# suyashk12/hipgp

Measured on NVIDIA B200. Metric: toeplitz_matvec_GBps_in_pcg_1e6grid, higher is better.
Workload: dtype f32

## Files before the change

hipgp_b200/csrc/conv_kernels.cuh:

```cuda
#pragma once
#include "fft_engine.cuh"

namespace hipgp {

enum RowsFwdMode { RF_PLAIN = 0, RF_PUPDATE = 1, RF_XRUPDATE = 2, RF_SELFDOT = 3 };
enum RowsInvMode { RI_PLAIN = 0, RI_DOT = 1 };
enum DotKind { DOT_PAP = 0, DOT_ZR = 1, DOT_RR = 2 };
enum ColsMode { CM_FWD = 0, CM_INV = 1, CM_FUSED = 2 };
enum SpecKind { SPEC_NONE = 0, SPEC_REAL = 1, SPEC_CPLX = 2, SPEC_CPLX_CONJ = 3 };

struct PcgDev {
    double* zr;
    double* zr_prev;
    double* pAp;
    double* rr;
    const double* rr_all;
    double* partial;
    unsigned* row_cnt;
    unsigned* rhs_cnt;
    int* flags;
    double tol;
    int B;
    int cg_mode;
};
// ... 33 lines not shown
                st.row_cnt[b] = 0;
                if (kind == DOT_PAP) st.pAp[b] = v;
                else if (kind == DOT_ZR) { st.zr_prev[b] = st.zr[b]; st.zr[b] = v; }
                else {
                    st.rr[b] = v;
                    if (st.cg_mode) { st.zr_prev[b] = st.zr[b]; st.zr[b] = v; }
                }
                __threadfence();
                if (kind == DOT_RR) {
                    const unsigned nb = atomicAdd(st.rhs_cnt, 1u) + 1u;
                    if (nb == (unsigned)st.B) {
                        __threadfence();
                        bool all = true;
                        const volatile double* rr = st.rr_all ? st.rr_all : st.rr;
                        for (int i = 0; i < st.B; ++i) all = all && (sqrt(rr[i]) < st.tol);
                        st.rhs_cnt[0] = 0;
                        st.flags[1] += 1;
                        st.flags[2] = 0;
                        if (all) st.flags[0] = 1;
                    }
                }
            }
        }
    }
}

template <class T>
struct RowsParams {
    const T* in;
    T* out;
    T* v0;
    T* v1;
    const T* v2;
    cplx<T>* W;
    long total_rows;
    int nrows;
    int n_real;
    int L, H;
    long W_pitch;
    int W_rows;
    LineFft<T> f;
    const cplx<T>* twL;
    const cplx<T>* twLp;
    const int* part;
    const int* pairq;
    const int* pairs; const cplx<T>* pairw; int npair0;
    const int* quadq; const cplx<T>* quadw; int nquad;
    int RB, RBP;
    int mode, dot_kind, do_fft;
    int vec_ok;
    int vec16_ok;
    int tma_ok;
    int tma_op;
    const void* spec; int spec_kind;
    PcgDev st;
};

template <class T>
__global__ void __launch_bounds__(256) rows_fwd_kernel(RowsParams<T> P) {
    HIPGP_DYN_SMEM(smem_raw);
    cplx<T>* s = reinterpret_cast<cplx<T>*>(smem_raw);
    const int tid = threadIdx.x, nthreads = blockDim.x;
    const int warp = tid >> 5, lane = tid & 31, nwarps = nthreads >> 5;
    if (P.mode != RF_PLAIN && P.st.flags[0]) return;
    const long g0 = (long)blockIdx.x * P.RB;
    const long g1 = g0 + P.RB < P.total_rows ? g0 + P.RB : P.total_rows;
    const int nl = (int)(g1 - g0);
    const int H = P.H, RBP = P.RBP, n = P.n_real;

    for (int line = warp; line < P.RB; line += nwarps) {
        if (line >= nl) {
            if (P.do_fft) for (int k = lane; k < H; k += 32) s[(size_t)k * RBP + line] = mk<T>(0, 0);
            continue;
        }
        const long g = g0 + line;
        const int b = (int)(g / P.nrows);
        const size_t off = (size_t)g * n;
        T acc = 0;
        T coef = 0;
        bool first = false;
        if (P.mode == RF_PUPDATE) {
            first = P.st.flags[2] != 0;
            coef = first ? (T)0 : (T)(P.st.zr[b] / P.st.zr_prev[b]);
        } else if (P.mode == RF_XRUPDATE) {
            coef = (T)(P.st.zr[b] / P.st.pAp[b]);
        }
        for (int k = lane; k < H; k += 32) {
            T e[2];
#pragma unroll
            for (int h = 0; h < 2; ++h) {
                const int i = 2 * k + h;
                T val = 0;
                if (i < n) {
                    if (P.mode == RF_PLAIN) {
                        val = P.in[off + i];
                    } else if (P.mode == RF_PUPDATE) {
                        const T z = P.in[off + i];
                        val = first ? z : z + coef * P.v0[off + i];
                        P.v0[off + i] = val;
                    } else if (P.mode == RF_SELFDOT) {
                        val = P.in[off + i];
                        acc += val * val;
                    } else {
                        const T pv = P.v2[off + i];
                        P.v1[off + i] = P.v1[off + i] + coef * pv;
                        val = P.v0[off + i] - coef * P.in[off + i];
// ... 193 lines not shown
```

hipgp_b200/csrc/fast_kernels.cuh:

```cuda
#pragma once
#include "lane_fft.cuh"

namespace hipgp {

template <class T> __device__ __forceinline__ void ld2(const T* p, bool vec, T& a, T& b, bool ok0, bool ok1) {
    if (vec && ok1) { const cplx<T> t = ld_stream(reinterpret_cast<const cplx<T>*>(p)); a = t.x; b = t.y; }
    else { a = ok0 ? ld_stream(p) : (T)0; b = ok1 ? ld_stream(p + 1) : (T)0; }
}
template <class T> __device__ __forceinline__ void st2(T* p, bool vec, T a, T b, bool ok0, bool ok1) {
    if (vec && ok1) { st_stream(reinterpret_cast<cplx<T>*>(p), mk<T>(a, b)); }
    else { if (ok0) st_stream(p, a); if (ok1) st_stream(p + 1, b); }
}

__device__ __forceinline__ double team_sum(double v, int tw) {
    for (int o = tw >> 1; o > 0; o >>= 1) v += __shfl_xor_sync(0xffffffffu, v, o);
    return v;
}

__device__ __forceinline__ Lane<float> lane_spec(Lane<float> v, const void* spec, int kind, size_t idx) {
    if (kind == SPEC_REAL) {
        const cplx<float> sv = ld_stream(reinterpret_cast<const cplx<float>*>(reinterpret_cast<const float*>(spec) + idx));
        return lmul_real2(v, sv.x, sv.y);
    }
    const cplx<float>* sp = reinterpret_cast<const cplx<float>*>(spec) + idx;
    const cplx<float> w0 = ld_stream(sp), w1 = ld_stream(sp + 1);
    return kind == SPEC_CPLX ? lmul_cplx2<false>(v, w0, w1) : lmul_cplx2<true>(v, w0, w1);
}
__device__ __forceinline__ Lane<double> lane_spec(Lane<double> v, const void* spec, int kind, size_t idx) {
    if (kind == SPEC_REAL) return lscale(v, ld_stream(reinterpret_cast<const double*>(spec) + idx));
    const cplx<double> w = ld_stream(reinterpret_cast<const cplx<double>*>(spec) + idx);
    return kind == SPEC_CPLX ? lmul(v, w) : lmulc(v, w);
}
__device__ __forceinline__ Lane<float> lane_spec_smem(Lane<float> v, const void* p) {
    const float2 s2 = *reinterpret_cast<const float2*>(p);
    Lane<float> r; r.re = __fmul2_rn(v.re, s2); r.im = __fmul2_rn(v.im, s2); return r;
}
__device__ __forceinline__ Lane<double> lane_spec_smem(Lane<double> v, const void* p) { return lscale(v, *reinterpret_cast<const double*>(p)); }

template <class T, int NL, int NT, int MINB, int R0, int... Rs>
__global__ void __launch_bounds__(NT, MINB) cols_fast_kernel(ColsParams<T> P) {
    using G = TileGeo<T, NL, R0, Rs...>;
    constexpr int Ln = G::Ln, NST = G::NST, RLAST = G::RLAST, LPT = LaneInfo<T>::LPT, TBL = NL * LPT, S0 = Ln / R0;
    HIPGP_DYN_SMEM(smem_raw);
    Lane<T>* s = reinterpret_cast<Lane<T>*>(smem_raw);
    const int tid = threadIdx.x;
    if (P.done_flag && *P.done_flag) return;
    const int mode = P.mode;
    const size_t pitch = (size_t)P.pitch;
    const size_t spitch = P.spec_pitch ? (size_t)P.spec_pitch : (size_t)P.pitch;
    const long ntiles = (long)P.nx * P.ny * P.nz;
    auto tile_origin = [&](long t, long& c0, size_t& ioff, size_t& ooff) {
        long bx, by, bz;
        if (P.batch_fastest) { bz = t % P.nz; const long r = t / P.nz; bx = r % P.nx; by = r / P.nx; }
        else { bx = t % P.nx; const long r = t / P.nx; by = r % P.ny; bz = r / P.ny; }
// ... 464 lines not shown
            if (tid < nl) { double a = 0.0; for (int k = 0; k < WPR; ++k) a += s_part[tid * WPR + k]; P.st.partial[g0 + tid] = a; }
        }
    }
    __syncthreads();
    if (want_dot) pcg_finalize(P.st, mode == RF_XRUPDATE ? DOT_RR : DOT_ZR, g0, g1, P.nrows, tid, NT);

    {
        const bool zero_hi = is_pow2(R0) && R0 > 1 && (n + 1) / 2 <= H / 2;
        const cplx<T>* tw0 = P.f.twst + P.f.twoff[0];
#pragma unroll 1
        for (int it = tid; it < S0 * NL; it += NT) {
            const int lane = it % NL, j = it / NL;
            cplx<T> w[R0];
            if (NST > 1) lane_twiddles<R0, S0>(w, tw0, j);
            const T* srow0 = side + (size_t)(lane * LPT) * SROW;
            const T* srow1 = side + (size_t)(lane * LPT + LPT - 1) * SROW;
            const bool ok0 = lane * LPT < nl, ok1 = lane * LPT + LPT - 1 < nl;
            auto elem = [&](int r) -> Lane<T> {
                const int i = 2 * (j + r * S0);
                const bool in_row = i < SROW;
                const cplx<T> e0 = (ok0 && in_row) ? *reinterpret_cast<const cplx<T>*>(srow0 + i) : mk<T>(0, 0);
                const cplx<T> e1 = (LPT == 2 && ok1 && in_row) ? *reinterpret_cast<const cplx<T>*>(srow1 + i) : mk<T>(0, 0);
                return lane_make(e0, e1);
            };
            Lane<T> v[R0];
            if (zero_hi) {
#pragma unroll
                for (int r = 0; r < R0 / 2; ++r) v[r] = elem(r);
                lbfly_zero_hi<R0, T>(v);
            } else {
#pragma unroll
                for (int r = 0; r < R0; ++r) v[r] = elem(r);
                lbfly<R0, false, T>(v);
            }
            if (NST > 1) {
#pragma unroll
                for (int r = 1; r < R0; ++r) v[r] = lmul(v[r], w[r]);
            }
            Lane<T>* base = s + (G::slot(j) * NL + lane);
#pragma unroll
            for (int r = 0; r < R0; ++r) base[r * LEG0] = v[r];
        }
    }
    __syncthreads();

    if constexpr (NST > 1) {
        LaneMidFwd<G, T, NL, NT, H / R0, 1, Rs...>::run(s, P.f, tid);
        lane_stage<G, T, NL, NT, RLAST, RLAST, false>(s, P.f.twst, tid);
        __syncthreads();
    }

    constexpr int NPAIR0 = NST > 1 ? RLAST / 2 + 1 : H / 2 + 1;
    constexpr int NQUAD = NST > 1 ? (H - RLAST) / 4 : 0;
#pragma unroll 1
    for (int it = tid; it < NPAIR0 * NL; it += NT) {
        const int lane = it % NL, pi = it / NL;
        const QuadIdx pq = reinterpret_cast<const QuadIdx*>(P.pairs)[pi];
        const int q = pq.a, q2 = pq.b;
        Lane<T> Xa, Xb;
        bool two;
        if (q == 0) {
            const Lane<T> z = s[lane];
            Lane<T> zs; zs.re = z.im; zs.im = z.re;
            Xa = lscale(z + zs, (T)2); Xb = lscale(z - zs, (T)2);
            Xa.im = lzero<T>().im; Xb.im = lzero<T>().im;
            two = true;
        } else {
            const cplx<T> wq = ldg_c(P.pairw + pi);
            const Lane<T> a = s[G::slot(q) * NL + lane], c = lconj(s[G::slot(q2) * NL + lane]);
            const Lane<T> E = a + c;
            const Lane<T> t = lmul(lmi<false>(a - c), wq);
            Xa = E + t; Xb = lconj(E - t);
            two = q2 != q;
        }
#pragma unroll
        for (int l = 0; l < LPT; ++l) {
            const int row = lane * LPT + l;
            if (row < nl) {
                cplx<T>* dst = P.W + s_wbase[row];
                WRow<T>::store1(dst, q, lane_get(Xa, l));
                if (two) WRow<T>::store1(dst, q2, lane_get(Xb, l));
            }
        }
    }
    if constexpr (NQUAD > 0) {
        constexpr int QIT = (NQUAD * NL + NT - 1) / NT;
        QuadIdx qq[QIT]; cplx<T> wa[QIT], wa1[QIT];
#pragma unroll
        for (int k = 0; k < QIT; ++k) {
            const int it = tid + k * NT, qi = it / NL;
            if (it < NQUAD * NL) { qq[k] = reinterpret_cast<const QuadIdx*>(P.quadq)[qi]; wa[k] = ldg_c(P.quadw + 2 * qi); wa1[k] = ldg_c(P.quadw + 2 * qi + 1); }
        }
#pragma unroll
        for (int k = 0; k < QIT; ++k) {
            const int it = tid + k * NT, lane = it % NL;
            if (it < NQUAD * NL) {
                const Lane<T>* pa = s + (G::slot(qq[k].a) * NL + lane);
                const Lane<T>* pb = s + (G::slot(qq[k].b) * NL + lane);
                const Lane<T> za = pa[0], za1 = pa[NL], zb = pb[0], zb1 = pb[NL];
                Lane<T> c = lconj(zb1);
                Lane<T> E = za + c;
                Lane<T> t = lmul(lmi<false>(za - c), wa[k]);
                const Lane<T> Xa = E + t, Xb1 = lconj(E - t);
                c = lconj(zb);
                E = za1 + c;
                t = lmul(lmi<false>(za1 - c), wa1[k]);
                const Lane<T> Xa1 = E + t, Xb = lconj(E - t);
                const bool self = qq[k].a == qq[k].b;
#pragma unroll
                for (int l = 0; l < LPT; ++l) {
                    const int row = lane * LPT + l;
                    if (row < nl) {
                        cplx<T>* dst = P.W + s_wbase[row];
                        if (self) WRow<T>::store2(dst, qq[k].a, lane_get(Xa, l), lane_get(Xb1, l));
                        else { WRow<T>::store2(dst, qq[k].a, lane_get(Xa, l), lane_get(Xa1, l)); WRow<T>::store2(dst, qq[k].b, lane_get(Xb, l), lane_get(Xb1, l)); }
                    }
                }
            }
        }
    }
#ifndef HIPGP_EMU
    if (bulk_store_pending && tid == 0) asm volatile("cp.async.bulk.wait_group.read 0;" ::: "memory");
#endif
}

template <class T, int NL, int NT, int MINB, int R0, int... Rs>
__global__ void __launch_bounds__(NT, MINB) rows_inv_fast_kernel(RowsParams<T> P) {
    using G = TileGeo<T, NL, R0, Rs...>;
    constexpr int H = G::Ln, NST = G::NST, RLAST = G::RLAST, LPT = LaneInfo<T>::LPT, NROW = NL * LPT, S0 = H / R0;
    constexpr int LEG0 = G::leg(NST > 1 ? S0 : 1);
    HIPGP_DYN_SMEM(smem_raw);
    Lane<T>* s = reinterpret_cast<Lane<T>*>(smem_raw);
    const int tid = threadIdx.x;
    if (P.mode != RI_PLAIN && P.st.flags[0]) return;
    const long g0 = (long)blockIdx.x * NROW;
    const long g1 = g0 + NROW < P.total_rows ? g0 + NROW : P.total_rows;
    const int nl = (int)(g1 - g0);
    const int n = P.n_real;

    __shared__ long s_wbase[32];
    __shared__ double s_part[32];
    if (tid < NROW && tid < nl) {
        const long gr = g0 + tid;
        const long b = gr / P.nrows;
        s_wbase[tid] = (b * P.W_rows + (gr - b * P.nrows)) * P.W_pitch;
    }
    __syncthreads();

    const int spec_kind = P.spec_kind;
    constexpr int NPAIR0 = NST > 1 ? RLAST / 2 + 1 : H / 2 + 1;
    constexpr int NQUAD = NST > 1 ? (H - RLAST) / 4 : 0;
#pragma unroll 1
    for (int it = tid; it < NPAIR0 * NL; it += NT) {
        const int lane = it % NL, pi = it / NL;
        const QuadIdx pq = reinterpret_cast<const QuadIdx*>(P.pairs)[pi];
        const int q = pq.a, q2 = pq.b;
        const cplx<T> wq = ldg_c(P.pairw + pi);
        cplx<T> ya[LPT], yc[LPT];
#pragma unroll
        for (int l = 0; l < LPT; ++l) {
            const int row = lane * LPT + l;
            ya[l] = mk<T>(0, 0); yc[l] = mk<T>(0, 0);
            if (row < nl) {
                const cplx<T>* src = P.W + s_wbase[row];
                ya[l] = WRow<T>::load1(src, q); yc[l] = WRow<T>::load1(src, q2);
                if (spec_kind != SPEC_NONE) { ya[l] = apply_spec(ya[l], P.spec, spec_kind, (size_t)q); yc[l] = apply_spec(yc[l], P.spec, spec_kind, (size_t)q2); }
            }
        }
        const Lane<T> a = lane_make(ya[0], ya[LPT - 1]);
        Lane<T> c = lane_make(yc[0], yc[LPT - 1]);
        if (q == 0) {
            Lane<T> z; z.re = (a + c).re; z.im = (a - c).re;
            s[lane] = z;
        } else {
            c = lconj(c);
            const Lane<T> E = a + c;
            const Lane<T> iO = lmi<true>(lmulc(a - c, wq));
            s[G::slot(q) * NL + lane] = E + iO;
            if (q2 != q) s[G::slot(q2) * NL + lane] = lconj(E - iO);
        }
    }
    if constexpr (NQUAD > 0) {
        constexpr int QIT = (NQUAD * NL + NT - 1) / NT;
        QuadIdx qq[QIT]; cplx<T> wa[QIT], wa1[QIT];
        cplx<T> ya[QIT][LPT], ya1[QIT][LPT], yb[QIT][LPT], yb1[QIT][LPT];
#pragma unroll
        for (int k = 0; k < QIT; ++k) {
            int it = tid + k * NT;
            it = it < NQUAD * NL ? it : NQUAD * NL - 1;
            const int qi = it / NL;
            qq[k] = reinterpret_cast<const QuadIdx*>(P.quadq)[qi]; wa[k] = ldg_c(P.quadw + 2 * qi); wa1[k] = ldg_c(P.quadw + 2 * qi + 1);
        }
#pragma unroll
        for (int k = 0; k < QIT; ++k) {
            int it = tid + k * NT;
            it = it < NQUAD * NL ? it : NQUAD * NL - 1;
            const int lane = it % NL;
#pragma unroll
            for (int l = 0; l < LPT; ++l) {
                const int row = lane * LPT + l;
                const cplx<T>* src = P.W + s_wbase[row < nl ? row : nl - 1];
                WRow<T>::load2(src, qq[k].a, ya[k][l], ya1[k][l]);
                WRow<T>::load2(src, qq[k].b, yb[k][l], yb1[k][l]);
            }
        }
#pragma unroll
        for (int k = 0; k < QIT; ++k) {
            const int it = tid + k * NT, lane = it % NL;
            if (it < NQUAD * NL) {
                const bool self = qq[k].a == qq[k].b;
                if (spec_kind != SPEC_NONE) {
#pragma unroll
                    for (int l = 0; l < LPT; ++l) {
                        ya[k][l] = apply_spec(ya[k][l], P.spec, spec_kind, (size_t)qq[k].a); ya1[k][l] = apply_spec(ya1[k][l], P.spec, spec_kind, (size_t)qq[k].a + 1);
                        yb[k][l] = apply_spec(yb[k][l], P.spec, spec_kind, (size_t)qq[k].b); yb1[k][l] = apply_spec(yb1[k][l], P.spec, spec_kind, (size_t)qq[k].b + 1);
                    }
                }
                const Lane<T> A = lane_make(ya[k][0], ya[k][LPT - 1]), A1 = lane_make(ya1[k][0], ya1[k][LPT - 1]);
                const Lane<T> Bn = lane_make(yb[k][0], yb[k][LPT - 1]), B1 = lane_make(yb1[k][0], yb1[k][LPT - 1]);
                Lane<T>* pa = s + (G::slot(qq[k].a) * NL + lane);
                Lane<T>* pb = s + (G::slot(qq[k].b) * NL + lane);
                Lane<T> c = lconj(B1);
                Lane<T> E = A + c;
                Lane<T> iO = lmi<true>(lmulc(A - c, wa[k]));
                pa[0] = E + iO;
                pb[NL] = lconj(E - iO);
                if (!self) {
                    c = lconj(Bn);
                    E = A1 + c;
                    iO = lmi<true>(lmulc(A1 - c, wa1[k]));
                    pa[NL] = E + iO;
                    pb[0] = lconj(E - iO);
                }
            }
        }
    }
    __syncthreads();

    if constexpr (NST > 1) {
        lane_stage<G, T, NL, NT, RLAST, RLAST, true>(s, P.f.twst, tid);
        __syncthreads();
        LaneMidInv<G, T, NL, NT, H / R0, 1, Rs...>::run(s, P.f, tid);
    }

    const int SROW = (n + 3) & ~3;
    T* side = reinterpret_cast<T*>(smem_raw + G::smem_bytes());
    const bool want_dot = P.mode == RI_DOT;
    {
        const bool out_lo = is_pow2(R0) && R0 > 1 && (n + 1) / 2 <= H / 2;
        const cplx<T>* tw0 = P.f.twst + P.f.twoff[0];
#pragma unroll 1
        for (int it = tid; it < S0 * NL; it += NT) {
            const int lane = it % NL, j = it / NL;
            cplx<T> w[R0];
            if (NST > 1) lane_twiddles<R0, S0>(w, tw0, j);
            const Lane<T>* base = s + (G::slot(j) * NL + lane);
            Lane<T> v[R0];
#pragma unroll
// ... 114 lines not shown
```

hipgp_b200/csrc/fast_launch.cuh:

```cuda
#pragma once
#include "plan_types.cuh"
#include "fast_kernels.cuh"
#include "cols_blk_kernel.cuh"

namespace hipgp {

constexpr int cfg_min(int a, int b) { return a < b ? a : b; }
constexpr int cfg_max(int a, int b) { return a > b ? a : b; }
constexpr int pow2_floor(int x) { return x <= 1 ? 1 : 2 * pow2_floor(x / 2); }

template <class T, int... Rs>
struct FastCfg {
    using List = RL<Rs...>;
    static constexpr int Ln = RLInfo<List>::N;
    static constexpr int RMAX = RLMax<List>::value;
    static constexpr int BFN = Ln / RMAX;
    static constexpr int NL0 = pow2_floor(cfg_max(1, cfg_min(256 / cfg_max(BFN, 1), 4096 / Ln)));
    static constexpr int NL = cfg_max(1, cfg_min(16, NL0));
    static constexpr int NT = cfg_min(512, cfg_max(32, (BFN * NL + 31) / 32 * 32));
    static constexpr int MINB = cfg_max(1, 512 / NT);
    static constexpr int LPT = LaneInfo<T>::LPT;
    static constexpr int S0 = Ln / (RLInfo<List>::count ? RLFirst<List>::value : 1);
    static constexpr int NLR = cfg_max(1, NL / 4);
    static constexpr int NTR = cfg_min(512, cfg_max(32, (BFN * NLR + 31) / 32 * 32));
    static constexpr int MINBR = cfg_max(1, 512 / NTR);
    static constexpr int RLASTv = RLLast<List>::value;
    static constexpr bool WIDEN = (NL == 1) && (RLInfo<List>::count > 1) && ((size_t)(Ln + Ln / RLASTv) * 2 * 24 <= 222 * 1024);
    static constexpr int CMULF = 2;
    static constexpr bool CMUL = !WIDEN && NL == 2 && ((size_t)(Ln + Ln / RLASTv) * NL * CMULF * 24 <= 222 * 1024) && BFN * NL * CMULF <= 512;
    static constexpr int NLC = WIDEN ? 2 : (CMUL ? NL * CMULF : NL);
    static constexpr int NTC = (WIDEN || CMUL) ? cfg_min(512, cfg_max(32, (BFN * NLC + 31) / 32 * 32)) : NT;
    static constexpr int MINBC = (WIDEN || CMUL) ? cfg_max(1, 512 / NTC) : MINB;
};

static void launch_check(const char* what, int len, int nl, int nt, size_t smem, long grid) {
    const cudaError_t e = cudaGetLastError();
    if (e != cudaSuccess)
        throw Error(std::string(what) + " launch failed (length " + std::to_string(len) + ", lanes " + std::to_string(nl) + ", threads " + std::to_string(nt) +
                    ", shared " + std::to_string(smem) + " B, grid " + std::to_string(grid) + "): " + cudaGetErrorString(e));
}

template <class T, int... Rs>
static void launch_rows_fast_t(hipgp_plan* pl, bool inverse, RowsParams<T>& P, cudaStream_t st) {
    using C = FastCfg<T, Rs...>;
    using G = TileGeo<T, C::NLR, Rs...>;
    constexpr int NROW = C::NLR * C::LPT;
    static_assert(NROW <= 32, "per-row scalars are held in 32-entry shared arrays");
    P.RB = NROW; P.RBP = NROW;
    {
        constexpr int NST = G::NST, H = C::Ln;
        const int want_q = NST > 1 ? (H - G::RLAST) / 4 : 0, want_p = NST > 1 ? G::RLAST / 2 + 1 : H / 2 + 1;
        if (P.nquad != want_q || P.npair0 != want_p) throw Error("internal: unexpected r2c pair structure for H = " + std::to_string(H));
    }
    const size_t smem = G::smem_bytes() + sizeof(T) * (size_t)((P.n_real + 3) & ~3) * NROW;
    if (smem > 227 * 1024) throw Error("row pass: rows too long for the shared-memory side buffer");
    static const char* env_nt = getenv("HIPGP_NO_TMA");
    static const char* env_nf = getenv("HIPGP_NO_TMA_FUSED");
    P.tma_ok = env_nt ? 0 : 1;
    P.tma_op = (!env_nf && !inverse && 2 * sizeof(T) * (size_t)((P.n_real + 3) & ~3) * NROW <= G::smem_bytes()) ? 1 : 0;
    dim3 grid((unsigned)((P.total_rows + NROW - 1) / NROW));
    PROF_BEGIN(pl, inverse ? 2 : 0, st);
    if (inverse) {
        auto k = rows_inv_fast_kernel<T, C::NLR, C::NTR, C::MINBR, Rs...>;
        if (smem > 40 * 1024) HIPGP_SET_MAX_SMEM(k, smem);
        HIPGP_LAUNCH(k, grid, dim3(C::NTR), smem, st, P);
    } else {
        auto k = rows_fwd_fast_kernel<T, C::NLR, C::NTR, C::MINBR, Rs...>;
        if (smem > 40 * 1024) HIPGP_SET_MAX_SMEM(k, smem);
        HIPGP_LAUNCH(k, grid, dim3(C::NTR), smem, st, P);
    }
    PROF_END(pl, st);
    launch_check("row pass", C::Ln, C::NLR, C::NTR, smem, (long)grid.x);
    pl->launches++;
}

template <class K>
static int resident_ctas(K kernel, int nthreads, size_t smem) {
#ifdef HIPGP_EMU
    (void)kernel; (void)nthreads; (void)smem;
    return 3;
#else
    int dev = 0, sms = 0, per = 0;
    CK(cudaGetDevice(&dev));
    CK(cudaDeviceGetAttribute(&sms, cudaDevAttrMultiProcessorCount, dev));
    CK(cudaOccupancyMaxActiveBlocksPerMultiprocessor(&per, kernel, nthreads, smem));
    return sms * (per > 0 ? per : 1);
#endif
}

template <class T, int LEN, int... Rs>
static void launch_cols_fast_t(hipgp_plan* pl, ColsParams<T>& P, long n_outer, long B, cudaStream_t st) {
    using C = FastCfg<T, Rs...>;
    using G = TileGeo<T, C::NLC, Rs...>;
    static_assert(C::Ln == LEN, "radix list does not multiply to the length");
    constexpr int TBL = C::NLC * C::LPT;
    P.TB = TBL; P.TBP = TBL;
    if ((P.in_split_len && (P.mode != CM_INV || P.in_split_len % G::RLAST)) || (P.out_split_len && (P.mode != CM_FWD || P.out_split_len % G::RLAST)))
        throw Error("split row blocks are supported for forward-only outputs / inverse-only inputs, in multiples of the last radix");
    const size_t side_bytes = G::NST > 1 ? (size_t)(C::Ln + C::Ln / G::RLAST) * C::NLC * 8 : 0;
    static const char* env_ns = getenv("HIPGP_NO_STAGE");
    const bool use_side = G::NST > 1 && !env_ns;
    P.spec_stage = (use_side && P.mode == CM_FUSED && P.spec_kind == SPEC_REAL) ? 1 : 0;
    P.in_stage = (use_side && P.mode != CM_INV && (size_t)P.n_in * C::NLC * 16 <= side_bytes) ? 1 : 0;
    const size_t smem = G::smem_bytes() + ((P.spec_stage || P.in_stage) ? side_bytes : 0);
    P.nx = (int)((P.inner + TBL - 1) / TBL); P.ny = (int)n_outer; P.nz = (int)B;
    {
        const size_t spec_bytes = (size_t)G::Ln * (size_t)P.inner * (P.spec_kind == SPEC_REAL ? sizeof(T) : 2 * sizeof(T));
        P.batch_fastest = (P.mode == CM_FUSED && B > 1 && spec_bytes > ((size_t)48 << 20) && (size_t)TBL * sizeof(cplx<T>) >= 128) ? 1 : 0;
    }
    auto k = cols_fast_kernel<T, C::NLC, C::NTC, C::MINBC, Rs...>;
    if (smem > 40 * 1024) HIPGP_SET_MAX_SMEM(k, smem);
    const long ntiles = (long)P.nx * P.ny * P.nz;
// ... 98 lines not shown
```

hipgp_b200/csrc/lane_fft.cuh:

```cuda
#pragma once
#include "conv_kernels.cuh"

namespace hipgp {

#ifdef HIPGP_EMU
static inline float2 __fadd2_rn(float2 a, float2 b) { return float2{a.x + b.x, a.y + b.y}; }
static inline float2 __fmul2_rn(float2 a, float2 b) { return float2{a.x * b.x, a.y * b.y}; }
static inline float2 __ffma2_rn(float2 a, float2 b, float2 c) { return float2{std::fma(a.x, b.x, c.x), std::fma(a.y, b.y, c.y)}; }
#endif

template <class T> struct Lane;
template <> struct __align__(16) Lane<float> { float2 re, im; };
template <> struct __align__(16) Lane<double> { double re, im; };
template <class T> struct LaneInfo { static constexpr int LPT = sizeof(T) == 4 ? 2 : 1; };

__device__ __forceinline__ float2 bc2(float s) { return make_float2(s, s); }
__device__ __forceinline__ float2 neg2(float2 a) { return make_float2(-a.x, -a.y); }

template <class T> __device__ __forceinline__ Lane<T> lzero();
template <> __device__ __forceinline__ Lane<float> lzero<float>() { Lane<float> r; r.re = bc2(0.f); r.im = bc2(0.f); return r; }
template <> __device__ __forceinline__ Lane<double> lzero<double>() { Lane<double> r; r.re = 0.0; r.im = 0.0; return r; }

__device__ __forceinline__ Lane<float> operator+(Lane<float> a, Lane<float> b) { Lane<float> r; r.re = __fadd2_rn(a.re, b.re); r.im = __fadd2_rn(a.im, b.im); return r; }
__device__ __forceinline__ Lane<float> operator-(Lane<float> a, Lane<float> b) { Lane<float> r; r.re = __fadd2_rn(a.re, neg2(b.re)); r.im = __fadd2_rn(a.im, neg2(b.im)); return r; }
// ... 83 lines not shown
__device__ __forceinline__ Lane<double> lane_from_global(const cplx<double>* p) {
#ifdef HIPGP_EMU
    return *reinterpret_cast<const Lane<double>*>(p);
#else
    const double2 t = __ldcg(reinterpret_cast<const double2*>(p));
    Lane<double> r; r.re = t.x; r.im = t.y; return r;
#endif
}
__device__ __forceinline__ void lane_to_global(cplx<float>* p, Lane<float> v) {
#ifdef HIPGP_EMU
    *reinterpret_cast<Lane<float>*>(p) = v;
#else
    __stcg(reinterpret_cast<float4*>(p), make_float4(v.re.x, v.re.y, v.im.x, v.im.y));
#endif
}
__device__ __forceinline__ void lane_to_global(cplx<double>* p, Lane<double> v) {
#ifdef HIPGP_EMU
    *reinterpret_cast<Lane<double>*>(p) = v;
#else
    __stcg(reinterpret_cast<double2*>(p), make_double2(v.re, v.im));
#endif
}

__device__ __forceinline__ float2 pack2(float a, float b) {
#ifdef HIPGP_EMU
    return make_float2(a, b);
#else
    unsigned long long r;
    asm("mov.b64 %0, {%1, %2};" : "=l"(r) : "f"(a), "f"(b));
    float2 o;
    asm("mov.b64 {%0, %1}, %2;" : "=f"(o.x), "=f"(o.y) : "l"(r));
    return o;
#endif
}
__device__ __forceinline__ Lane<float> lane_make(cplx<float> v0, cplx<float> v1) { Lane<float> r; r.re = pack2(v0.x, v1.x); r.im = pack2(v0.y, v1.y); return r; }
__device__ __forceinline__ Lane<double> lane_make(cplx<double> v0, cplx<double>) { Lane<double> r; r.re = v0.x; r.im = v0.y; return r; }

template <class T> struct WRow;
template <> struct WRow<float> {
    static __device__ __forceinline__ void store1(cplx<float>* row, int q, cplx<float> v) {
        float* f = reinterpret_cast<float*>(row) + 4 * (q >> 1) + (q & 1); st_stream(f, v.x); st_stream(f + 2, v.y);
    }
    static __device__ __forceinline__ cplx<float> load1(const cplx<float>* row, int q) {
        const float* f = reinterpret_cast<const float*>(row) + 4 * (q >> 1) + (q & 1); return mk<float>(ld_stream(f), ld_stream(f + 2));
    }
    static __device__ __forceinline__ void store2(cplx<float>* row, int q, cplx<float> v0, cplx<float> v1) {
        Lane<float> t; t.re = make_float2(v0.x, v1.x); t.im = make_float2(v0.y, v1.y);
        lane_to_global(row + q, t);
    }
    static __device__ __forceinline__ void load2(const cplx<float>* row, int q, cplx<float>& v0, cplx<float>& v1) {
        const Lane<float> t = lane_from_global(row + q);
        v0 = mk<float>(t.re.x, t.im.x); v1 = mk<float>(t.re.y, t.im.y);
    }
};
template <> struct WRow<double> {
    static __device__ __forceinline__ void store1(cplx<double>* row, int q, cplx<double> v) { st_stream(row + q, v); }
    static __device__ __forceinline__ cplx<double> load1(const cplx<double>* row, int q) { return ld_stream(row + q); }
    static __device__ __forceinline__ void store2(cplx<double>* row, int q, cplx<double> v0, cplx<double> v1) { st_stream(row + q, v0); st_stream(row + q + 1, v1); }
    static __device__ __forceinline__ void load2(const cplx<double>* row, int q, cplx<double>& v0, cplx<double>& v1) { v0 = ld_stream(row + q); v1 = ld_stream(row + q + 1); }
};

template <int BYTES> __device__ __forceinline__ void cp_async(void* smem_dst, const void* gmem_src) {
#ifdef HIPGP_EMU
    std::memcpy(smem_dst, gmem_src, BYTES);
#else
    const unsigned sa = (unsigned)__cvta_generic_to_shared(smem_dst);
    if (BYTES == 16) asm volatile("cp.async.cg.shared.global [%0], [%1], 16;" ::"r"(sa), "l"(gmem_src));
    else asm volatile("cp.async.ca.shared.global [%0], [%1], 8;" ::"r"(sa), "l"(gmem_src));
#endif
}
__device__ __forceinline__ void cp_async_commit() {
#ifndef HIPGP_EMU
    asm volatile("cp.async.commit_group;" ::: "memory");
#endif
}
__device__ __forceinline__ void cp_async_wait_all() {
#ifndef HIPGP_EMU
    asm volatile("cp.async.wait_group 0;" ::: "memory");
#endif
}

#ifndef HIPGP_EMU
__device__ __forceinline__ void mbar_init(unsigned long long* bar, unsigned count) {
    asm volatile("mbarrier.init.shared::cta.b64 [%0], %1;" ::"r"((unsigned)__cvta_generic_to_shared(bar)), "r"(count) : "memory");
}
__device__ __forceinline__ void fence_proxy_async() { asm volatile("fence.proxy.async.shared::cta;" ::: "memory"); }
__device__ __forceinline__ void mbar_arrive_expect_tx(unsigned long long* bar, unsigned bytes) {
    asm volatile("mbarrier.arrive.expect_tx.shared::cta.b64 _, [%0], %1;" ::"r"((unsigned)__cvta_generic_to_shared(bar)), "r"(bytes) : "memory");
}
__device__ __forceinline__ void mbar_wait(unsigned long long* bar, unsigned parity) {
    const unsigned a = (unsigned)__cvta_generic_to_shared(bar);
    asm volatile(
        "{\n\t.reg .pred P1;\n\t"
        "HIPGP_MBAR_WAIT:\n\t"
        "mbarrier.try_wait.parity.shared::cta.b64 P1, [%0], %1, 0x989680;\n\t"
        "@P1 bra HIPGP_MBAR_DONE;\n\t"
        "bra HIPGP_MBAR_WAIT;\n\t"
        "HIPGP_MBAR_DONE:\n\t}" ::"r"(a), "r"(parity) : "memory");
}
__device__ __forceinline__ void bulk_g2s(void* smem_dst, const void* gmem_src, unsigned bytes, unsigned long long* bar) {
    asm volatile("cp.async.bulk.shared::cluster.global.mbarrier::complete_tx::bytes [%0], [%1], %2, [%3];"
                 ::"r"((unsigned)__cvta_generic_to_shared(smem_dst)), "l"(gmem_src), "r"(bytes), "r"((unsigned)__cvta_generic_to_shared(bar)) : "memory");
}
__device__ __forceinline__ void bulk_s2g(void* gmem_dst, const void* smem_src, unsigned bytes) {
    asm volatile("cp.async.bulk.global.shared::cta.bulk_group [%0], [%1], %2;" ::"l"(gmem_dst), "r"((unsigned)__cvta_generic_to_shared(smem_src)), "r"(bytes) : "memory");
    asm volatile("cp.async.bulk.commit_group;" ::: "memory");
    asm volatile("cp.async.bulk.wait_group.read 0;" ::: "memory");
}
__device__ __forceinline__ void bulk_s2g_issue(void* gmem_dst, const void* smem_src, unsigned bytes) {
    asm volatile("cp.async.bulk.global.shared::cta.bulk_group [%0], [%1], %2;" ::"l"(gmem_dst), "r"((unsigned)__cvta_generic_to_shared(smem_src)), "r"(bytes) : "memory");
    asm volatile("cp.async.bulk.commit_group;" ::: "memory");
}
// ... 208 lines not shown
```

hipgp_b200/csrc/tma_maps.cuh:

```cuda
#pragma once
#include "lane_fft.cuh"
#ifndef HIPGP_EMU
#include <cuda.h>
#endif

namespace hipgp {

#ifdef HIPGP_EMU
struct alignas(64) TensorMap3 {
    const unsigned char* base; unsigned long long dim[3]; unsigned long long stride[2]; unsigned box[3]; unsigned esize; int valid;
};
#define HIPGP_GRID_CONSTANT
#else
typedef CUtensorMap TensorMap3;
#define HIPGP_GRID_CONSTANT __grid_constant__
#endif

struct alignas(64) ColsTmaMaps { TensorMap3 in; TensorMap3 spec; };

static inline bool encode_map3(TensorMap3* out, const void* base, int esize, const unsigned long long dim[3],
                               const unsigned long long stride_bytes[2], const unsigned box[3]) {
#ifdef HIPGP_EMU
    out->base = (const unsigned char*)base; out->esize = (unsigned)esize; out->valid = 1;
    for (int i = 0; i < 3; ++i) { out->dim[i] = dim[i]; out->box[i] = box[i]; }
// ... 50 lines not shown
#ifndef HIPGP_EMU
    mbar_init(bar, 1);
#else
    (void)bar;
#endif
}
__device__ __forceinline__ void tma_bar_expect(unsigned long long* bar, unsigned bytes) {
#ifndef HIPGP_EMU
    mbar_arrive_expect_tx(bar, bytes);
#else
    (void)bar; (void)bytes;
#endif
}
__device__ __forceinline__ void tma_bar_wait(unsigned long long* bar, unsigned parity, int emu_id, int emu_count) {
#ifndef HIPGP_EMU
    (void)emu_id; (void)emu_count;
    mbar_wait(bar, parity);
#else
    (void)bar; (void)parity;
    emu::g_named_barrier[emu_id].sync(emu_count);
#endif
}
__device__ __forceinline__ void warps_bar_init(unsigned long long* bar, unsigned count) {
#ifndef HIPGP_EMU
    mbar_init(bar, count);
#else
    (void)bar; (void)count;
#endif
}
__device__ __forceinline__ void warps_bar_arrive(unsigned long long* bar, int emu_id, int count) {
#ifndef HIPGP_EMU
    (void)emu_id; (void)count;
    asm volatile("mbarrier.arrive.shared::cta.b64 _, [%0];" ::"r"((unsigned)__cvta_generic_to_shared(bar)) : "memory");
#else
    (void)bar;
    emu::g_named_barrier[emu_id].arrive(count);
#endif
}
__device__ __forceinline__ void warps_bar_arrive_and_wait(unsigned long long* bar, unsigned parity, int emu_id, int count) {
#ifndef HIPGP_EMU
    (void)emu_id; (void)count;
    asm volatile("mbarrier.arrive.shared::cta.b64 _, [%0];" ::"r"((unsigned)__cvta_generic_to_shared(bar)) : "memory");
    mbar_wait(bar, parity);
#else
    (void)bar; (void)parity;
    emu::g_named_barrier[emu_id].sync(count);
#endif
}
__device__ __forceinline__ void tma_fence_before_issue() {
#ifndef HIPGP_EMU
    fence_proxy_async();
#endif
}

}
```

Baseline: 450.7.

## Stage W rows in shared memory and move them with bulk TMA copies

```diff
diff --git a/hipgp_b200/csrc/conv_kernels.cuh b/hipgp_b200/csrc/conv_kernels.cuh
--- a/hipgp_b200/csrc/conv_kernels.cuh
+++ b/hipgp_b200/csrc/conv_kernels.cuh
@@ -109,6 +109,7 @@
     int vec16_ok;
     int tma_ok;
     int tma_op;
+    int tma_w;
     const void* spec; int spec_kind;
     PcgDev st;
 };
diff --git a/hipgp_b200/csrc/fast_kernels.cuh b/hipgp_b200/csrc/fast_kernels.cuh
--- a/hipgp_b200/csrc/fast_kernels.cuh
+++ b/hipgp_b200/csrc/fast_kernels.cuh
@@ -1,5 +1,6 @@
 #pragma once
 #include "lane_fft.cuh"
+#include "tma_maps.cuh"
 
 namespace hipgp {
 
@@ -570,75 +571,188 @@
 
     constexpr int NPAIR0 = NST > 1 ? RLAST / 2 + 1 : H / 2 + 1;
     constexpr int NQUAD = NST > 1 ? (H - RLAST) / 4 : 0;
-#pragma unroll 1
-    for (int it = tid; it < NPAIR0 * NL; it += NT) {
-        const int lane = it % NL, pi = it / NL;
-        const QuadIdx pq = reinterpret_cast<const QuadIdx*>(P.pairs)[pi];
-        const int q = pq.a, q2 = pq.b;
-        Lane<T> Xa, Xb;
-        bool two;
-        if (q == 0) {
-            const Lane<T> z = s[lane];
-            Lane<T> zs; zs.re = z.im; zs.im = z.re;
-            Xa = lscale(z + zs, (T)2); Xb = lscale(z - zs, (T)2);
-            Xa.im = lzero<T>().im; Xb.im = lzero<T>().im;
-            two = true;
-        } else {
-            const cplx<T> wq = ldg_c(P.pairw + pi);
-            const Lane<T> a = s[G::slot(q) * NL + lane], c = lconj(s[G::slot(q2) * NL + lane]);
-            const Lane<T> E = a + c;
-            const Lane<T> t = lmul(lmi<false>(a - c), wq);
-            Xa = E + t; Xb = lconj(E - t);
-            two = q2 != q;
-        }
-#pragma unroll
-        for (int l = 0; l < LPT; ++l) {
-            const int row = lane * LPT + l;
-            if (row < nl) {
-                cplx<T>* dst = P.W + s_wbase[row];
-                WRow<T>::store1(dst, q, lane_get(Xa, l));
-                if (two) WRow<T>::store1(dst, q2, lane_get(Xb, l));
-            }
-        }
-    }
-    if constexpr (NQUAD > 0) {
-        constexpr int QIT = (NQUAD * NL + NT - 1) / NT;
-        QuadIdx qq[QIT]; cplx<T> wa[QIT], wa1[QIT];
-#pragma unroll
-        for (int k = 0; k < QIT; ++k) {
-            const int it = tid + k * NT, qi = it / NL;
-            if (it < NQUAD * NL) { qq[k] = reinterpret_cast<const QuadIdx*>(P.quadq)[qi]; wa[k] = ldg_c(P.quadw + 2 * qi); wa1[k] = ldg_c(P.quadw + 2 * qi + 1); }
-        }
-#pragma unroll
-        for (int k = 0; k < QIT; ++k) {
+    const bool wst = P.tma_w != 0;
+    if (wst) {
+        const long wp = P.W_pitch;
+        cplx<T>* wsm = reinterpret_cast<cplx<T>*>(smem_raw);
+        constexpr int PIT = (NPAIR0 * NL + NT - 1) / NT;
+        constexpr int QIT = NQUAD > 0 ? (NQUAD * NL + NT - 1) / NT : 1;
+        QuadIdx pq[PIT]; cplx<T> pw[PIT]; Lane<T> pza[PIT], pzb[PIT];
+        QuadIdx qq[QIT]; cplx<T> wa[QIT], wa1[QIT]; Lane<T> za[QIT], za1[QIT], zb[QIT], zb1[QIT];
+#pragma unroll
+        for (int k = 0; k < PIT; ++k) {
+            const int it = tid + k * NT;
+            if (it < NPAIR0 * NL) { pq[k] = reinterpret_cast<const QuadIdx*>(P.pairs)[it / NL]; pw[k] = ldg_c(P.pairw + it / NL); }
+        }
+        if constexpr (NQUAD > 0) {
+#pragma unroll
+            for (int k = 0; k < QIT; ++k) {
+                const int it = tid + k * NT, qi = it / NL;
+                if (it < NQUAD * NL) { qq[k] = reinterpret_cast<const QuadIdx*>(P.quadq)[qi]; wa[k] = ldg_c(P.quadw + 2 * qi); wa1[k] = ldg_c(P.quadw + 2 * qi + 1); }
+            }
+        }
+#pragma unroll
+        for (int k = 0; k < PIT; ++k) {
             const int it = tid + k * NT, lane = it % NL;
-            if (it < NQUAD * NL) {
-                const Lane<T>* pa = s + (G::slot(qq[k].a) * NL + lane);
-                const Lane<T>* pb = s + (G::slot(qq[k].b) * NL + lane);
-                const Lane<T> za = pa[0], za1 = pa[NL], zb = pb[0], zb1 = pb[NL];
-                Lane<T> c = lconj(zb1);
-                Lane<T> E = za + c;
-                Lane<T> t = lmul(lmi<false>(za - c), wa[k]);
-                const Lane<T> Xa = E + t, Xb1 = lconj(E - t);
-                c = lconj(zb);
-                E = za1 + c;
-                t = lmul(lmi<false>(za1 - c), wa1[k]);
-                const Lane<T> Xa1 = E + t, Xb = lconj(E - t);
-                const bool self = qq[k].a == qq[k].b;
+            if (it < NPAIR0 * NL) {
+                if (pq[k].a == 0) pza[k] = s[lane];
+                else { pza[k] = s[G::slot(pq[k].a) * NL + lane]; pzb[k] = s[G::slot(pq[k].b) * NL + lane]; }
+            }
+        }
+        if constexpr (NQUAD > 0) {
+#pragma unroll
+            for (int k = 0; k < QIT; ++k) {
+                const int it = tid + k * NT, lane = it % NL;
+                if (it < NQUAD * NL) {
+                    const Lane<T>* pa = s + (G::slot(qq[k].a) * NL + lane);
+                    const Lane<T>* pb = s + (G::slot(qq[k].b) * NL + lane);
+                    za[k] = pa[0]; za1[k] = pa[NL]; zb[k] = pb[0]; zb1[k] = pb[NL];
+                }
+            }
+        }
+        __syncthreads();
+#pragma unroll
+        for (int k = 0; k < PIT; ++k) {
+            const int it = tid + k * NT, lane = it % NL;
+            if (it < NPAIR0 * NL) {
+                const int q = pq[k].a, q2 = pq[k].b;
+                Lane<T> Xa, Xb;
+                bool two;
+                if (q == 0) {
+                    const Lane<T> z = pza[k];
+                    Lane<T> zs; zs.re = z.im; zs.im = z.re;
+                    Xa = lscale(z + zs, (T)2); Xb = lscale(z - zs, (T)2);
+                    Xa.im = lzero<T>().im; Xb.im = lzero<T>().im;
+                    two = true;
+                } else {
+                    const Lane<T> a = pza[k], c = lconj(pzb[k]);
+                    const Lane<T> E = a + c;
+                    const Lane<T> t = lmul(lmi<false>(a - c), pw[k]);
+                    Xa = E + t; Xb = lconj(E - t);
+                    two = q2 != q;
+                }
 #pragma unroll
                 for (int l = 0; l < LPT; ++l) {
                     const int row = lane * LPT + l;
                     if (row < nl) {
-                        cplx<T>* dst = P.W + s_wbase[row];
-                        if (self) WRow<T>::store2(dst, qq[k].a, lane_get(Xa, l), lane_get(Xb1, l));
-                        else { WRow<T>::store2(dst, qq[k].a, lane_get(Xa, l), lane_get(Xa1, l)); WRow<T>::store2(dst, qq[k].b, lane_get(Xb, l), lane_get(Xb1, l)); }
+                        WRow<T>::sts1(wsm + row * wp, q, lane_get(Xa, l));
+                        if (two) WRow<T>::sts1(wsm + row * wp, q2, lane_get(Xb, l));
+                    }
+                }
+            }
+        }
+        if constexpr (NQUAD > 0) {
+#pragma unroll
+            for (int k = 0; k < QIT; ++k) {
+                const int it = tid + k * NT, lane = it % NL;
+                if (it < NQUAD * NL) {
+                    Lane<T> c = lconj(zb1[k]);
+                    Lane<T> E = za[k] + c;
+                    Lane<T> t = lmul(lmi<false>(za[k] - c), wa[k]);
+                    const Lane<T> Xa = E + t, Xb1 = lconj(E - t);
+                    c = lconj(zb[k]);
+                    E = za1[k] + c;
+                    t = lmul(lmi<false>(za1[k] - c), wa1[k]);
+                    const Lane<T> Xa1 = E + t, Xb = lconj(E - t);
+                    const bool self = qq[k].a == qq[k].b;
+#pragma unroll
+                    for (int l = 0; l < LPT; ++l) {
+                        const int row = lane * LPT + l;
+                        if (row < nl) {
+                            cplx<T>* dst = wsm + row * wp;
+                            if (self) WRow<T>::sts2(dst, qq[k].a, lane_get(Xa, l), lane_get(Xb1, l));
+                            else { WRow<T>::sts2(dst, qq[k].a, lane_get(Xa, l), lane_get(Xa1, l)); WRow<T>::sts2(dst, qq[k].b, lane_get(Xb, l), lane_get(Xb1, l)); }
+                        }
+                    }
+                }
+            }
+        }
+        {
+            const int npad = (int)(wp - H - 1);
+            for (int i = tid; i < nl * npad; i += NT) WRow<T>::sts1(wsm + (i / npad) * wp, H + 1 + i % npad, mk<T>(0, 0));
+        }
+        tma_fence_before_issue();
+        __syncthreads();
+        if (tid == 0) {
+            const unsigned rbytes = (unsigned)((size_t)wp * sizeof(cplx<T>));
+            long b = g0 / P.nrows, r = g0 - b * P.nrows;
+            for (int i = 0; i < nl; ++i) {
+                bulk_store(P.W + (b * P.W_rows + r) * wp, wsm + i * wp, rbytes);
+                if (++r == P.nrows) { r = 0; ++b; }
+            }
+            bulk_store_commit();
+        }
+    } else {
+#pragma unroll 1
+        for (int it = tid; it < NPAIR0 * NL; it += NT) {
+            const int lane = it % NL, pi = it / NL;
+            const QuadIdx pq = reinterpret_cast<const QuadIdx*>(P.pairs)[pi];
+            const int q = pq.a, q2 = pq.b;
+            Lane<T> Xa, Xb;
+            bool two;
+            if (q == 0) {
+                const Lane<T> z = s[lane];
+                Lane<T> zs; zs.re = z.im; zs.im = z.re;
+                Xa = lscale(z + zs, (T)2); Xb = lscale(z - zs, (T)2);
+                Xa.im = lzero<T>().im; Xb.im = lzero<T>().im;
+                two = true;
+            } else {
+                const cplx<T> wq = ldg_c(P.pairw + pi);
+                const Lane<T> a = s[G::slot(q) * NL + lane], c = lconj(s[G::slot(q2) * NL + lane]);
+                const Lane<T> E = a + c;
+                const Lane<T> t = lmul(lmi<false>(a - c), wq);
+                Xa = E + t; Xb = lconj(E - t);
+                two = q2 != q;
+            }
+#pragma unroll
+            for (int l = 0; l < LPT; ++l) {
+                const int row = lane * LPT + l;
+                if (row < nl) {
+                    cplx<T>* dst = P.W + s_wbase[row];
+                    WRow<T>::store1(dst, q, lane_get(Xa, l));
+                    if (two) WRow<T>::store1(dst, q2, lane_get(Xb, l));
+                }
+            }
+        }
+        if constexpr (NQUAD > 0) {
+            constexpr int QIT = (NQUAD * NL + NT - 1) / NT;
+            QuadIdx qq[QIT]; cplx<T> wa[QIT], wa1[QIT];
+#pragma unroll
+            for (int k = 0; k < QIT; ++k) {
+                const int it = tid + k * NT, qi = it / NL;
+                if (it < NQUAD * NL) { qq[k] = reinterpret_cast<const QuadIdx*>(P.quadq)[qi]; wa[k] = ldg_c(P.quadw + 2 * qi); wa1[k] = ldg_c(P.quadw + 2 * qi + 1); }
+            }
+#pragma unroll
+            for (int k = 0; k < QIT; ++k) {
+                const int it = tid + k * NT, lane = it % NL;
+                if (it < NQUAD * NL) {
+                    const Lane<T>* pa = s + (G::slot(qq[k].a) * NL + lane);
+                    const Lane<T>* pb = s + (G::slot(qq[k].b) * NL + lane);
+                    const Lane<T> za = pa[0], za1 = pa[NL], zb = pb[0], zb1 = pb[NL];
+                    Lane<T> c = lconj(zb1);
+                    Lane<T> E = za + c;
+                    Lane<T> t = lmul(lmi<false>(za - c), wa[k]);
+                    const Lane<T> Xa = E + t, Xb1 = lconj(E - t);
+                    c = lconj(zb);
+                    E = za1 + c;
+                    t = lmul(lmi<false>(za1 - c), wa1[k]);
+                    const Lane<T> Xa1 = E + t, Xb = lconj(E - t);
+                    const bool self = qq[k].a == qq[k].b;
+#pragma unroll
+                    for (int l = 0; l < LPT; ++l) {
+                        const int row = lane * LPT + l;
+                        if (row < nl) {
+                            cplx<T>* dst = P.W + s_wbase[row];
+                            if (self) WRow<T>::store2(dst, qq[k].a, lane_get(Xa, l), lane_get(Xb1, l));
+                            else { WRow<T>::store2(dst, qq[k].a, lane_get(Xa, l), lane_get(Xa1, l)); WRow<T>::store2(dst, qq[k].b, lane_get(Xb, l), lane_get(Xb1, l)); }
+                        }
                     }
                 }
             }
         }
     }
 #ifndef HIPGP_EMU
-    if (bulk_store_pending && tid == 0) asm volatile("cp.async.bulk.wait_group.read 0;" ::: "memory");
+    if ((bulk_store_pending || wst) && tid == 0) asm volatile("cp.async.bulk.wait_group.read 0;" ::: "memory");
 #endif
 }
 
@@ -650,7 +764,6 @@
     HIPGP_DYN_SMEM(smem_raw);
     Lane<T>* s = reinterpret_cast<Lane<T>*>(smem_raw);
     const int tid = threadIdx.x;
-    if (P.mode != RI_PLAIN && P.st.flags[0]) return;
     const long g0 = (long)blockIdx.x * NROW;
     const long g1 = g0 + NROW < P.total_rows ? g0 + NROW : P.total_rows;
     const int nl = (int)(g1 - g0);
@@ -658,7 +771,28 @@
 
     __shared__ long s_wbase[32];
     __shared__ double s_part[32];
-    if (tid < NROW && tid < nl) {
+    __shared__ unsigned long long s_wbar;
+    const bool wst = P.tma_w != 0;
+    const long wp = P.W_pitch;
+    const cplx<T>* wsm = reinterpret_cast<const cplx<T>*>(smem_raw);
+    if (wst && tid == 0) {
+        tma_bar_init(&s_wbar);
+        tma_fence_before_issue();
+        const unsigned rbytes = (unsigned)((size_t)wp * sizeof(cplx<T>));
+        tma_bar_expect(&s_wbar, rbytes * (unsigned)nl);
+        long b = g0 / P.nrows, r = g0 - b * P.nrows;
+        for (int i = 0; i < nl; ++i) {
+            bulk_load(smem_raw + (size_t)i * rbytes, P.W + (b * P.W_rows + r) * wp, rbytes, &s_wbar);
+            if (++r == P.nrows) { r = 0; ++b; }
+        }
+    }
+    if (P.mode != RI_PLAIN && P.st.flags[0]) {
+#ifndef HIPGP_EMU
+        if (wst && tid == 0) mbar_wait(&s_wbar, 0);
+#endif
+        return;
+    }
+    if (!wst && tid < NROW && tid < nl) {
         const long gr = g0 + tid;
         const long b = gr / P.nrows;
         s_wbase[tid] = (b * P.W_rows + (gr - b * P.nrows)) * P.W_pitch;
@@ -668,22 +802,11 @@
     const int spec_kind = P.spec_kind;
     constexpr int NPAIR0 = NST > 1 ? RLAST / 2 + 1 : H / 2 + 1;
     constexpr int NQUAD = NST > 1 ? (H - RLAST) / 4 : 0;
-#pragma unroll 1
-    for (int it = tid; it < NPAIR0 * NL; it += NT) {
-        const int lane = it % NL, pi = it / NL;
-        const QuadIdx pq = reinterpret_cast<const QuadIdx*>(P.pairs)[pi];
-        const int q = pq.a, q2 = pq.b;
-        const cplx<T> wq = ldg_c(P.pairw + pi);
-        cplx<T> ya[LPT], yc[LPT];
-#pragma unroll
-        for (int l = 0; l < LPT; ++l) {
-            const int row = lane * LPT + l;
-            ya[l] = mk<T>(0, 0); yc[l] = mk<T>(0, 0);
-            if (row < nl) {
-                const cplx<T>* src = P.W + s_wbase[row];
-                ya[l] = WRow<T>::load1(src, q); yc[l] = WRow<T>::load1(src, q2);
-                if (spec_kind != SPEC_NONE) { ya[l] = apply_spec(ya[l], P.spec, spec_kind, (size_t)q); yc[l] = apply_spec(yc[l], P.spec, spec_kind, (size_t)q2); }
-            }
+    auto merge_pair = [&](int lane, int q, int q2, cplx<T> wq, cplx<T>* ya, cplx<T>* yc) {
+        if (spec_kind != SPEC_NONE) {
+#pragma unroll
+            for (int l = 0; l < LPT; ++l)
+                if (lane * LPT + l < nl) { ya[l] = apply_spec(ya[l], P.spec, spec_kind, (size_t)q); yc[l] = apply_spec(yc[l], P.spec, spec_kind, (size_t)q2); }
         }
         const Lane<T> a = lane_make(ya[0], ya[LPT - 1]);
         Lane<T> c = lane_make(yc[0], yc[LPT - 1]);
@@ -697,11 +820,11 @@
             s[G::slot(q) * NL + lane] = E + iO;
             if (q2 != q) s[G::slot(q2) * NL + lane] = lconj(E - iO);
         }
-    }
-    if constexpr (NQUAD > 0) {
-        constexpr int QIT = (NQUAD * NL + NT - 1) / NT;
-        QuadIdx qq[QIT]; cplx<T> wa[QIT], wa1[QIT];
-        cplx<T> ya[QIT][LPT], ya1[QIT][LPT], yb[QIT][LPT], yb1[QIT][LPT];
+    };
+    constexpr int QIT = NQUAD > 0 ? (NQUAD * NL + NT - 1) / NT : 1;
+    QuadIdx qq[QIT]; cplx<T> wa[QIT], wa1[QIT];
+    cplx<T> ya[QIT][LPT], ya1[QIT][LPT], yb[QIT][LPT], yb1[QIT][LPT];
+    auto load_quad_tables = [&]() {
 #pragma unroll
         for (int k = 0; k < QIT; ++k) {
             int it = tid + k * NT;
@@ -709,19 +832,87 @@
             const int qi = it / NL;
             qq[k] = reinterpret_cast<const QuadIdx*>(P.quadq)[qi]; wa[k] = ldg_c(P.quadw + 2 * qi); wa1[k] = ldg_c(P.quadw + 2 * qi + 1);
         }
-#pragma unroll
-        for (int k = 0; k < QIT; ++k) {
-            int it = tid + k * NT;
-            it = it < NQUAD * NL ? it : NQUAD * NL - 1;
-            const int lane = it % NL;
+    };
+    if (wst) {
+        constexpr int PIT = (NPAIR0 * NL + NT - 1) / NT;
+        QuadIdx pq[PIT]; cplx<T> pw[PIT], pya[PIT][LPT], pyc[PIT][LPT];
+#pragma unroll
+        for (int k = 0; k < PIT; ++k) {
+            const int it = tid + k * NT;
+            if (it < NPAIR0 * NL) { pq[k] = reinterpret_cast<const QuadIdx*>(P.pairs)[it / NL]; pw[k] = ldg_c(P.pairw + it / NL); }
+        }
+        if constexpr (NQUAD > 0) load_quad_tables();
+        tma_bar_wait(&s_wbar, 0, 0, NT);
+#pragma unroll
+        for (int k = 0; k < PIT; ++k) {
+            const int it = tid + k * NT, lane = it % NL;
+            if (it < NPAIR0 * NL) {
+#pragma unroll
+                for (int l = 0; l < LPT; ++l) {
+                    const int row = lane * LPT + l;
+                    pya[k][l] = mk<T>(0, 0); pyc[k][l] = mk<T>(0, 0);
+                    if (row < nl) { pya[k][l] = WRow<T>::lds1(wsm + row * wp, pq[k].a); pyc[k][l] = WRow<T>::lds1(wsm + row * wp, pq[k].b); }
+                }
+            }
+        }
+        if constexpr (NQUAD > 0) {
+#pragma unroll
+            for (int k = 0; k < QIT; ++k) {
+                int it = tid + k * NT;
+                it = it < NQUAD * NL ? it : NQUAD * NL - 1;
+                const int lane = it % NL;
+#pragma unroll
+                for (int l = 0; l < LPT; ++l) {
+                    const int row = lane * LPT + l;
+                    const cplx<T>* src = wsm + (row < nl ? row : nl - 1) * wp;
+                    WRow<T>::lds2(src, qq[k].a, ya[k][l], ya1[k][l]);
+                    WRow<T>::lds2(src, qq[k].b, yb[k][l], yb1[k][l]);
+                }
+            }
+        }
+        __syncthreads();
+#pragma unroll
+        for (int k = 0; k < PIT; ++k) {
+            const int it = tid + k * NT;
+            if (it < NPAIR0 * NL) merge_pair(it % NL, pq[k].a, pq[k].b, pw[k], pya[k], pyc[k]);
+        }
+    } else {
+#pragma unroll 1
+        for (int it = tid; it < NPAIR0 * NL; it += NT) {
+            const int lane = it % NL, pi = it / NL;
+            const QuadIdx pq = reinterpret_cast<const QuadIdx*>(P.pairs)[pi];
+            const int q = pq.a, q2 = pq.b;
+            const cplx<T> wq = ldg_c(P.pairw + pi);
+            cplx<T> pya[LPT], pyc[LPT];
 #pragma unroll
             for (int l = 0; l < LPT; ++l) {
                 const int row = lane * LPT + l;
-                const cplx<T>* src = P.W + s_wbase[row < nl ? row : nl - 1];
-                WRow<T>::load2(src, qq[k].a, ya[k][l], ya1[k][l]);
-                WRow<T>::load2(src, qq[k].b, yb[k][l], yb1[k][l]);
-            }
-        }
+                pya[l] = mk<T>(0, 0); pyc[l] = mk<T>(0, 0);
+                if (row < nl) {
+                    const cplx<T>* src = P.W + s_wbase[row];
+                    pya[l] = WRow<T>::load1(src, q); pyc[l] = WRow<T>::load1(src, q2);
+                }
+            }
+            merge_pair(lane, q, q2, wq, pya, pyc);
+        }
+        if constexpr (NQUAD > 0) {
+            load_quad_tables();
+#pragma unroll
+            for (int k = 0; k < QIT; ++k) {
+                int it = tid + k * NT;
+                it = it < NQUAD * NL ? it : NQUAD * NL - 1;
+                const int lane = it % NL;
+#pragma unroll
+                for (int l = 0; l < LPT; ++l) {
+                    const int row = lane * LPT + l;
+                    const cplx<T>* src = P.W + s_wbase[row < nl ? row : nl - 1];
+                    WRow<T>::load2(src, qq[k].a, ya[k][l], ya1[k][l]);
+                    WRow<T>::load2(src, qq[k].b, yb[k][l], yb1[k][l]);
+                }
+            }
+        }
+    }
+    if constexpr (NQUAD > 0) {
 #pragma unroll
         for (int k = 0; k < QIT; ++k) {
             const int it = tid + k * NT, lane = it % NL;
diff --git a/hipgp_b200/csrc/fast_launch.cuh b/hipgp_b200/csrc/fast_launch.cuh
--- a/hipgp_b200/csrc/fast_launch.cuh
+++ b/hipgp_b200/csrc/fast_launch.cuh
@@ -58,6 +58,10 @@
     static const char* env_nf = getenv("HIPGP_NO_TMA_FUSED");
     P.tma_ok = env_nt ? 0 : 1;
     P.tma_op = (!env_nf && !inverse && 2 * sizeof(T) * (size_t)((P.n_real + 3) & ~3) * NROW <= G::smem_bytes()) ? 1 : 0;
+    static const char* env_nw = getenv("HIPGP_NO_TMA_W");
+    const size_t wrow_bytes = (size_t)P.W_pitch * sizeof(cplx<T>);
+    P.tma_w = (P.tma_ok && !env_nw && (inverse || sizeof(T) == 4) && (size_t)NROW * wrow_bytes <= G::smem_bytes() &&
+               (uintptr_t)P.W % 16 == 0 && wrow_bytes % 16 == 0) ? 1 : 0;
     dim3 grid((unsigned)((P.total_rows + NROW - 1) / NROW));
     PROF_BEGIN(pl, inverse ? 2 : 0, st);
     if (inverse) {
diff --git a/hipgp_b200/csrc/lane_fft.cuh b/hipgp_b200/csrc/lane_fft.cuh
--- a/hipgp_b200/csrc/lane_fft.cuh
+++ b/hipgp_b200/csrc/lane_fft.cuh
@@ -159,12 +159,30 @@
         const Lane<float> t = lane_from_global(row + q);
         v0 = mk<float>(t.re.x, t.im.x); v1 = mk<float>(t.re.y, t.im.y);
     }
+    static __device__ __forceinline__ void sts1(cplx<float>* row, int q, cplx<float> v) {
+        float* f = reinterpret_cast<float*>(row) + 4 * (q >> 1) + (q & 1); f[0] = v.x; f[2] = v.y;
+    }
+    static __device__ __forceinline__ cplx<float> lds1(const cplx<float>* row, int q) {
+        const float* f = reinterpret_cast<const float*>(row) + 4 * (q >> 1) + (q & 1); return mk<float>(f[0], f[2]);
+    }
+    static __device__ __forceinline__ void sts2(cplx<float>* row, int q, cplx<float> v0, cplx<float> v1) {
+        Lane<float> t; t.re = make_float2(v0.x, v1.x); t.im = make_float2(v0.y, v1.y);
+        *reinterpret_cast<Lane<float>*>(row + q) = t;
+    }
+    static __device__ __forceinline__ void lds2(const cplx<float>* row, int q, cplx<float>& v0, cplx<float>& v1) {
+        const Lane<float> t = *reinterpret_cast<const Lane<float>*>(row + q);
+        v0 = mk<float>(t.re.x, t.im.x); v1 = mk<float>(t.re.y, t.im.y);
+    }
 };
 template <> struct WRow<double> {
     static __device__ __forceinline__ void store1(cplx<double>* row, int q, cplx<double> v) { st_stream(row + q, v); }
     static __device__ __forceinline__ cplx<double> load1(const cplx<double>* row, int q) { return ld_stream(row + q); }
     static __device__ __forceinline__ void store2(cplx<double>* row, int q, cplx<double> v0, cplx<double> v1) { st_stream(row + q, v0); st_stream(row + q + 1, v1); }
     static __device__ __forceinline__ void load2(const cplx<double>* row, int q, cplx<double>& v0, cplx<double>& v1) { v0 = ld_stream(row + q); v1 = ld_stream(row + q + 1); }
+    static __device__ __forceinline__ void sts1(cplx<double>* row, int q, cplx<double> v) { row[q] = v; }
+    static __device__ __forceinline__ cplx<double> lds1(const cplx<double>* row, int q) { return row[q]; }
+    static __device__ __forceinline__ void sts2(cplx<double>* row, int q, cplx<double> v0, cplx<double> v1) { row[q] = v0; row[q + 1] = v1; }
+    static __device__ __forceinline__ void lds2(const cplx<double>* row, int q, cplx<double>& v0, cplx<double>& v1) { v0 = row[q]; v1 = row[q + 1]; }
 };
 
 template <int BYTES> __device__ __forceinline__ void cp_async(void* smem_dst, const void* gmem_src) {
diff --git a/hipgp_b200/csrc/tma_maps.cuh b/hipgp_b200/csrc/tma_maps.cuh
--- a/hipgp_b200/csrc/tma_maps.cuh
+++ b/hipgp_b200/csrc/tma_maps.cuh
@@ -126,5 +126,25 @@
     fence_proxy_async();
 #endif
 }
+__device__ __forceinline__ void bulk_load(void* smem_dst, const void* gmem_src, unsigned bytes, unsigned long long* bar) {
+#ifndef HIPGP_EMU
+    bulk_g2s(smem_dst, gmem_src, bytes, bar);
+#else
+    (void)bar;
+    std::memcpy(smem_dst, gmem_src, bytes);
+#endif
+}
+__device__ __forceinline__ void bulk_store(void* gmem_dst, const void* smem_src, unsigned bytes) {
+#ifndef HIPGP_EMU
+    asm volatile("cp.async.bulk.global.shared::cta.bulk_group [%0], [%1], %2;" ::"l"(gmem_dst), "r"((unsigned)__cvta_generic_to_shared(smem_src)), "r"(bytes) : "memory");
+#else
+    std::memcpy(gmem_dst, smem_src, bytes);
+#endif
+}
+__device__ __forceinline__ void bulk_store_commit() {
+#ifndef HIPGP_EMU
+    asm volatile("cp.async.bulk.commit_group;" ::: "memory");
+#endif
+}
 
 }
```

Result: faster. 478.6 (median of 6 runs) (+6.2%).
